# praveer13/zest

Measured on AMD Instinct MI355X. Metric: aggregate pull GB/s + P2P ratio, Llama-3.1-70B at 1/2/4/8 MI355X peers, higher is better.
Workload: dtype bf16

## Files before the change

### csrc/gpu/compress.hip

```cpp
#include <hip/hip_runtime.h>

#include <cstdint>
#include <cstdlib>

#include "zgpu.h"

namespace {

constexpr int kWave = 64;
constexpr int kWavesPerBlock = 4;
constexpr int kTabLog = 12;
constexpr uint32_t kTab = 1u << kTabLog;

__device__ __forceinline__ uint32_t lane_id() { return threadIdx.x & (kWave - 1); }

__device__ __forceinline__ uint32_t load_u32(const uint8_t* p) {
  const uintptr_t a = reinterpret_cast<uintptr_t>(p);
  const uint32_t k = uint32_t(a & 3);
  const uint32_t* w = reinterpret_cast<const uint32_t*>(a & ~uintptr_t(3));
  const uint32_t w0 = w[0];
  return k == 0 ? w0 : __builtin_amdgcn_alignbyte(w[1], w0, k);
}

__device__ __forceinline__ uint32_t put_len(uint8_t* o, uint32_t op, uint32_t r, uint32_t lane) {
  const uint32_t nff = r / 255;
  for (uint32_t i = lane; i < nff; i += kWave) o[op + i] = 0xFF;
  if (lane == 0) o[op + nff] = uint8_t(r - 255 * nff);
  return op + nff + 1;
}

__device__ __forceinline__ uint32_t emit(uint8_t* o, uint32_t op, const uint8_t* in, uint32_t lit0, uint32_t L,
                                         uint32_t off, uint32_t ml, uint32_t lane) {
  const uint32_t M = ml ? ml - 4 : 0;
  if (lane == 0) o[op] = uint8_t(((L < 15 ? L : 15) << 4) | (ml ? (M < 15 ? M : 15) : 0));
  ++op;
  if (L >= 15) op = put_len(o, op, L - 15, lane);
  for (uint32_t i = lane; i < L; i += kWave) o[op + i] = in[lit0 + i];
  op += L;
  if (ml) {
    if (lane == 0) {
      o[op] = uint8_t(off & 0xFF);
      o[op + 1] = uint8_t(off >> 8);
    }
    op += 2;
    if (M >= 15) op = put_len(o, op, M - 15, lane);
  }
  return op;
}

__global__ void __launch_bounds__(256) k_bg4_split(const uint8_t* __restrict__ data, const uint64_t* __restrict__ offs,
                                                   const uint32_t* __restrict__ lens, int n, uint8_t* __restrict__ out,
                                                   uint64_t slot) {
  const int c = __builtin_amdgcn_readfirstlane(int(blockIdx.x * kWavesPerBlock + (threadIdx.x >> 6)));
  if (c >= n) return;
  const uint32_t lane = lane_id(), len = lens[c];
  const uint8_t* s = data + offs[c];
  uint8_t* d = out + uint64_t(c) * slot;
  const uint32_t q = len >> 2, r = len & 3;
  const uint32_t g1 = q + (r > 0), g2 = g1 + q + (r > 1), g3 = g2 + q + (r > 2);
  for (uint32_t i = lane; i < len; i += kWave) {
    const uint32_t g = i & 3, j = i >> 2;
    const uint32_t base = g == 0 ? 0u : g == 1 ? g1 : g == 2 ? g2 : g3;
    d[base + j] = s[i];
  }
}

__global__ void __launch_bounds__(256) k_lz4_compress_v1(const uint8_t* __restrict__ data, const uint64_t* __restrict__ offs,
                                                      const uint32_t* __restrict__ lens, int n, uint64_t in_slot,
                                                      uint8_t* __restrict__ out, uint64_t out_slot,
                                                      uint32_t* __restrict__ out_len, uint32_t hc64, uint32_t hc256) {
  __shared__ unsigned long long tabs[kWavesPerBlock][kTab];
  const int wave = __builtin_amdgcn_readfirstlane(int(threadIdx.x >> 6));
  const int c = __builtin_amdgcn_readfirstlane(int(blockIdx.x * kWavesPerBlock + wave));
  if (c >= n) return;
  const uint32_t lane = lane_id();
  unsigned long long* tab = tabs[wave];
  for (uint32_t i = lane; i < kTab; i += kWave) tab[i] = 0;
  __builtin_amdgcn_wave_barrier();
  const uint32_t len = lens[c];
  const uint8_t* in = in_slot ? data + uint64_t(c) * in_slot : data + offs[c];
  uint8_t* o = out + uint64_t(c) * out_slot;
  uint32_t op = 11, ip = 0, anchor = 0;
  const uint32_t mend = len > 5 ? len - 5 : 0;
  while (ip + 12 <= len) {
    const uint32_t p = ip + lane;
    const bool ok = p + 12 <= len;
    const uint32_t v = ok ? load_u32(in + p) : 0;
    const uint32_t h = (v * 2654435761u) >> (32 - kTabLog);
    const unsigned long long e = ok ? tab[h] : 0ull;
    uint32_t cand = uint32_t(e >> 32) - 1;
    bool hit = ok && e != 0 && uint32_t(e) == v && cand < p && p - cand <= 65535u;
    uint32_t near = 0;
    for (int d = 32; d >= 1; --d) {
      const uint32_t u = __shfl_up(v, d, kWave);
      if (lane >= uint32_t(d) && u == v) near = d;
    }
    if (ok && near) {
      cand = p - near;
      hit = true;
    }
    const unsigned long long mask = __ballot(hit);
    const uint32_t passed = mask ? uint32_t(__builtin_ctzll(mask)) + 1 : uint32_t(kWave);
    __builtin_amdgcn_wave_barrier();
    if (ok && lane < passed) atomicMax(&tab[h], (static_cast<unsigned long long>(p + 1) << 32) | v);
    if (!mask) {
      ip += kWave;
      continue;
    }
    const int j = __builtin_ctzll(mask);
    uint32_t mp = ip + uint32_t(j);
    uint32_t mc = uint32_t(__builtin_amdgcn_readlane(int(cand), j));
    while (true) {
      const uint32_t room = (mp - anchor) < mc ? (mp - anchor) : mc;
      if (room == 0) break;
      const uint32_t k = lane + 1;
      const bool eq = k <= room && in[mp - k] == in[mc - k];
      const unsigned long long ne = __ballot(!eq);
      const uint32_t b = ne ? uint32_t(__builtin_ctzll(ne)) : uint32_t(kWave);
      mp -= b;
      mc -= b;
      if (b < uint32_t(kWave)) break;
    }
    const uint32_t maxlen = mend - mp;
    uint32_t ml = 4 + (ip + uint32_t(j) - mp);
    while (ml < maxlen) {
      const uint32_t k = ml + lane;
      const bool eq = k < maxlen && in[mc + k] == in[mp + k];
      const unsigned long long ne = __ballot(!eq);
      if (ne) {
        ml += uint32_t(__builtin_ctzll(ne));
        break;
      }
      ml += kWave;
    }
    if (ml > maxlen) ml = maxlen;
    op = emit(o, op, in, anchor, mp - anchor, mp - mc, ml, lane);
    ip = mp + ml;
    anchor = ip;
  }
  op = emit(o, op, in, anchor, len - anchor, 0, 0, lane);
  const uint32_t total = op + 4;
  if (total >= len) {
    if (lane == 0) out_len[c] = 0;
    return;
  }
  if (lane == 0) {
    const uint32_t bs = op - 11;
    const bool small = len <= 65536;
    const uint8_t hdr[11] = {0x04, 0x22, 0x4D, 0x18, 0x60, uint8_t(small ? 0x40 : 0x50),
                             uint8_t(small ? hc64 : hc256), uint8_t(bs), uint8_t(bs >> 8), uint8_t(bs >> 16),
                             uint8_t(bs >> 24)};
    for (int i = 0; i < 11; ++i) o[i] = hdr[i];
    for (int i = 0; i < 4; ++i) o[op + i] = 0;
    out_len[c] = total;
  }
}

constexpr uint32_t kTagBits = 14;
constexpr uint32_t kTagMask = (1u << kTagBits) - 1;
constexpr uint32_t kRing = 4096;
constexpr uint32_t kRingMask = kRing - 1;
constexpr uint32_t kFlush = 2048;
constexpr uint32_t kHdr = 11;

struct Staged {
  uint8_t* ring;
  uint8_t* g;
  uint32_t flushed;
};

__device__ __forceinline__ void ring_write(Staged& o, uint32_t end, uint32_t lane) {
  __builtin_amdgcn_wave_barrier();
  for (uint32_t pos = o.flushed + lane; pos < end; pos += kWave)
    if (pos >= kHdr) o.g[pos] = o.ring[pos & kRingMask];
  __builtin_amdgcn_wave_barrier();
}

__device__ __forceinline__ void maybe_flush(Staged& o, uint32_t op, uint32_t lane) {
  while (op - o.flushed >= kFlush) {
    ring_write(o, o.flushed + kFlush, lane);
    o.flushed += kFlush;
  }
}

__device__ __forceinline__ uint32_t put_len_s(Staged& o, uint32_t op, uint32_t r, uint32_t lane) {
  const uint32_t nff = r / 255;
  for (uint32_t i = lane; i < nff; i += kWave) o.ring[(op + i) & kRingMask] = 0xFF;
  if (lane == 0) o.ring[(op + nff) & kRingMask] = uint8_t(r - 255 * nff);
  return op + nff + 1;
}

__device__ __forceinline__ uint32_t emit_s(Staged& o, uint32_t op, const uint8_t* in, uint32_t lit0, uint32_t L,
                                           uint32_t off, uint32_t ml, uint32_t lane) {
  const uint32_t M = ml ? ml - 4 : 0;
  maybe_flush(o, op, lane);
  if (lane == 0) o.ring[op & kRingMask] = uint8_t(((L < 15 ? L : 15) << 4) | (ml ? (M < 15 ? M : 15) : 0));
  ++op;
  if (L >= 15) op = put_len_s(o, op, L - 15, lane);
  for (uint32_t b = 0; b < L; b += 1024) {
    maybe_flush(o, op + b, lane);
    const uint32_t n = L - b < 1024 ? L - b : 1024;
    for (uint32_t i = lane; i < n; i += kWave) o.ring[(op + b + i) & kRingMask] = in[lit0 + b + i];
  }
  op += L;
  if (ml) {
    maybe_flush(o, op, lane);
    if (lane == 0) {
      o.ring[op & kRingMask] = uint8_t(off & 0xFF);
      o.ring[(op + 1) & kRingMask] = uint8_t(off >> 8);
    }
    op += 2;
    if (M >= 15) op = put_len_s(o, op, M - 15, lane);
  }
  return op;
}

__global__ void __launch_bounds__(256) k_lz4_compress(const uint8_t* __restrict__ data, const uint64_t* __restrict__ offs,
                                                      const uint32_t* __restrict__ lens, int n, uint64_t in_slot,
                                                      uint8_t* __restrict__ out, uint64_t out_slot,
                                                      uint32_t* __restrict__ out_len, uint32_t hc64, uint32_t hc256) {
  __shared__ uint32_t tabs[kWavesPerBlock][kTab];
  __shared__ uint8_t rings[kWavesPerBlock][kRing];
  const int wave = __builtin_amdgcn_readfirstlane(int(threadIdx.x >> 6));
  const int c = __builtin_amdgcn_readfirstlane(int(blockIdx.x * kWavesPerBlock + wave));
  if (c >= n) return;
  const uint32_t lane = lane_id();
  uint32_t* tab = tabs[wave];
  for (uint32_t i = lane; i < kTab; i += kWave) tab[i] = 0;
  __builtin_amdgcn_wave_barrier();
  const uint32_t len = lens[c];
  const uint8_t* in = in_slot ? data + uint64_t(c) * in_slot : data + offs[c];
  Staged o{rings[wave], out + uint64_t(c) * out_slot, 0};
  uint32_t op = kHdr, ip = 0, anchor = 0;
  const uint32_t mend = len > 5 ? len - 5 : 0;
  while (ip + 12 <= len) {
    const uint32_t p = ip + lane;
    const bool ok = p + 12 <= len;
    const uint32_t v = ok ? load_u32(in + p) : 0;
    const uint32_t hv = v * 2654435761u;
    const uint32_t h = hv >> (32 - kTabLog);
    const uint32_t tag = hv & kTagMask;
    const uint32_t e = ok ? tab[h] : 0u;
    uint32_t cand = (e >> kTagBits) - 1;
    bool hit = ok && e != 0 && (e & kTagMask) == tag && cand < p && p - cand <= 65535u;
    if (hit) hit = load_u32(in + cand) == v;
    uint32_t near = 0;
    for (int d = 32; d >= 1; --d) {
      const uint32_t u = __shfl_up(v, d, kWave);
      if (lane >= uint32_t(d) && u == v) near = d;
    }
    if (ok && near) {
      cand = p - near;
      hit = true;
    }
    const unsigned long long mask = __ballot(hit);
    const uint32_t passed = mask ? uint32_t(__builtin_ctzll(mask)) + 1 : uint32_t(kWave);
    __builtin_amdgcn_wave_barrier();
    if (ok && lane < passed) atomicMax(&tab[h], ((p + 1) << kTagBits) | tag);
    if (!mask) {
      ip += kWave;
      continue;
    }
    const int j = __builtin_ctzll(mask);
    uint32_t mp = ip + uint32_t(j);
    uint32_t mc = uint32_t(__builtin_amdgcn_readlane(int(cand), j));
    while (true) {
      const uint32_t room = (mp - anchor) < mc ? (mp - anchor) : mc;
      if (room == 0) break;
      const uint32_t k = lane + 1;
      const bool eq = k <= room && in[mp - k] == in[mc - k];
      const unsigned long long ne = __ballot(!eq);
      const uint32_t b = ne ? uint32_t(__builtin_ctzll(ne)) : uint32_t(kWave);
      mp -= b;
      mc -= b;
      if (b < uint32_t(kWave)) break;
    }
    const uint32_t maxlen = mend - mp;
    uint32_t ml = 4 + (ip + uint32_t(j) - mp);
    while (ml < maxlen) {
      const uint32_t k = ml + lane;
      const bool eq = k < maxlen && in[mc + k] == in[mp + k];
      const unsigned long long ne = __ballot(!eq);
      if (ne) {
        ml += uint32_t(__builtin_ctzll(ne));
        break;
      }
      ml += kWave;
    }
    if (ml > maxlen) ml = maxlen;
    op = emit_s(o, op, in, anchor, mp - anchor, mp - mc, ml, lane);
    ip = mp + ml;
    anchor = ip;
  }
  op = emit_s(o, op, in, anchor, len - anchor, 0, 0, lane);
  const uint32_t total = op + 4;
  if (total >= len) {
    if (lane == 0) out_len[c] = 0;
    return;
  }
  maybe_flush(o, op, lane);
  if (lane < 4) o.ring[(op + lane) & kRingMask] = 0;
  ring_write(o, total, lane);
  if (lane == 0) {
    const uint32_t bs = op - kHdr;
    const bool small = len <= 65536;
    const uint8_t hdr[kHdr] = {0x04, 0x22, 0x4D, 0x18, 0x60, uint8_t(small ? 0x40 : 0x50),
                               uint8_t(small ? hc64 : hc256), uint8_t(bs), uint8_t(bs >> 8), uint8_t(bs >> 16),
                               uint8_t(bs >> 24)};
    for (uint32_t i = 0; i < kHdr; ++i) o.g[i] = hdr[i];
    out_len[c] = total;
  }
}

bool compress_v1() {
  const char* e = getenv("ZG_COMPRESS");
  return e && e[0] == 'v' && e[1] == '1';
}

__global__ void __launch_bounds__(256) k_pack_frames(const uint64_t* __restrict__ src, const uint32_t* __restrict__ clen,
                                                     const uint32_t* __restrict__ ulen, const uint8_t* __restrict__ scheme,
                                                     const uint64_t* __restrict__ out_off, int n, uint8_t* __restrict__ out) {
  const int c = __builtin_amdgcn_readfirstlane(int(blockIdx.x * kWavesPerBlock + (threadIdx.x >> 6)));
  if (c >= n) return;
  const uint32_t lane = lane_id(), cl = clen[c], ul = ulen[c];
  uint8_t* d = out + out_off[c];
  if (lane < 8) {
    const uint32_t b = lane == 0 ? 0u : lane < 4 ? (cl >> (8 * (lane - 1))) & 0xFF
                                  : lane == 4 ? scheme[c] : (ul >> (8 * (lane - 5))) & 0xFF;
    d[lane] = uint8_t(b);
  }
  const uint8_t* s = reinterpret_cast<const uint8_t*>(src[c]);
  for (uint32_t i = lane; i < cl; i += kWave) d[8 + i] = s[i];
}

}

extern "C" {

hipError_t zg_compress_chunks(const uint8_t* data, const uint64_t* offs, const uint32_t* lens, int n, int bg4,
                              uint8_t* scratch, uint64_t in_slot, uint8_t* out, uint64_t out_slot, uint32_t* out_len,
                              uint32_t hc64, uint32_t hc256, hipStream_t stream) {
  if (n <= 0) return hipSuccess;
  const dim3 grid((n + kWavesPerBlock - 1) / kWavesPerBlock);
  auto* kern = compress_v1() ? k_lz4_compress_v1 : k_lz4_compress;
  if (bg4) {
    hipLaunchKernelGGL(k_bg4_split, grid, dim3(256), 0, stream, data, offs, lens, n, scratch, in_slot);
    hipLaunchKernelGGL(kern, grid, dim3(256), 0, stream, scratch, offs, lens, n, in_slot, out, out_slot, out_len,
                       hc64, hc256);
  } else {
    hipLaunchKernelGGL(kern, grid, dim3(256), 0, stream, data, offs, lens, n, uint64_t(0), out, out_slot, out_len,
                       hc64, hc256);
  }
  return hipGetLastError();
}

hipError_t zg_pack_frames(const uint64_t* src, const uint32_t* clen, const uint32_t* ulen, const uint8_t* scheme,
                          const uint64_t* out_off, int n, uint8_t* out, hipStream_t stream) {
  if (n <= 0) return hipSuccess;
  hipLaunchKernelGGL(k_pack_frames, dim3((n + kWavesPerBlock - 1) / kWavesPerBlock), dim3(256), 0, stream, src, clen,
                     ulen, scheme, out_off, n, out);
  return hipGetLastError();
}

}
```

Baseline: 63.18.

## Stage LZ4 input in LDS window, reuse wave scans after matches, vectorize byte-group split

```diff
diff --git a/csrc/gpu/compress.hip b/csrc/gpu/compress.hip
--- a/csrc/gpu/compress.hip
+++ b/csrc/gpu/compress.hip
@@ -48,6 +48,11 @@
   return op;
 }
 
+typedef uint32_t __attribute__((aligned(1))) dword_any;
+struct __attribute__((packed, aligned(1))) Dwords4 {
+  uint32_t v[4];
+};
+
 __global__ void __launch_bounds__(256) k_bg4_split(const uint8_t* __restrict__ data, const uint64_t* __restrict__ offs,
                                                    const uint32_t* __restrict__ lens, int n, uint8_t* __restrict__ out,
                                                    uint64_t slot) {
@@ -58,7 +63,18 @@
   uint8_t* d = out + uint64_t(c) * slot;
   const uint32_t q = len >> 2, r = len & 3;
   const uint32_t g1 = q + (r > 0), g2 = g1 + q + (r > 1), g3 = g2 + q + (r > 2);
-  for (uint32_t i = lane; i < len; i += kWave) {
+  const uint32_t nv = len >> 4;
+  for (uint32_t t = lane; t < nv; t += kWave) {
+    const Dwords4 a = *reinterpret_cast<const Dwords4*>(s + 16 * t);
+#pragma unroll
+    for (uint32_t g = 0; g < 4; ++g) {
+      const uint32_t base = g == 0 ? 0u : g == 1 ? g1 : g == 2 ? g2 : g3;
+      const uint32_t x = ((a.v[0] >> (8 * g)) & 0xFF) | (((a.v[1] >> (8 * g)) & 0xFF) << 8) |
+                         (((a.v[2] >> (8 * g)) & 0xFF) << 16) | (((a.v[3] >> (8 * g)) & 0xFF) << 24);
+      *reinterpret_cast<dword_any*>(d + base + 4 * t) = x;
+    }
+  }
+  for (uint32_t i = 16 * nv + lane; i < len; i += kWave) {
     const uint32_t g = i & 3, j = i >> 2;
     const uint32_t base = g == 0 ? 0u : g == 1 ? g1 : g == 2 ? g2 : g3;
     d[base + j] = s[i];
@@ -158,20 +174,135 @@
 
 constexpr uint32_t kTagBits = 14;
 constexpr uint32_t kTagMask = (1u << kTagBits) - 1;
-constexpr uint32_t kRing = 4096;
+constexpr uint32_t kRing = 2048;
 constexpr uint32_t kRingMask = kRing - 1;
-constexpr uint32_t kFlush = 2048;
+constexpr uint32_t kFlush = 1024;
+constexpr uint32_t kPiece = 512;
 constexpr uint32_t kHdr = 11;
+constexpr uint32_t kWin = 2048;
+constexpr uint32_t kWinDw = kWin / 4;
+constexpr uint32_t kBlk = 1024;
+constexpr uint32_t kAhead = 96;
+
+struct Win {
+  uint32_t* w;
+  const uint32_t* g;
+  uint32_t nd;
+  uint32_t lo, hi;
+  uint32_t pre[4];
+};
+
+__device__ __forceinline__ uint32_t glob_dw(const Win& s, int32_t d) {
+  const int32_t last = int32_t(s.nd) - 1;
+  const int32_t k = d < 0 ? 0 : d > last ? last : d;
+  const uint32_t x = *reinterpret_cast<const uint32_t*>(reinterpret_cast<const uint8_t*>(s.g) + (uint32_t(k) << 2));
+  return k == d ? x : 0u;
+}
+
+__device__ __forceinline__ uint32_t glob_u32(const Win& s, uint32_t q) {
+  const int32_t d = int32_t(q >> 2);
+  return __builtin_amdgcn_alignbyte(glob_dw(s, d + 1), glob_dw(s, d), q & 3);
+}
+
+__device__ __forceinline__ uint32_t glob_u8(const Win& s, uint32_t q) {
+  return (glob_dw(s, int32_t(q >> 2)) >> (8 * (q & 3))) & 0xFF;
+}
+
+__device__ __forceinline__ uint32_t win_dw(const Win& s, uint32_t d) { return s.w[d & (kWinDw - 1)]; }
+
+__device__ __forceinline__ uint32_t win_u32(const Win& s, uint32_t q) {
+  const uint32_t d = q >> 2;
+  return __builtin_amdgcn_alignbyte(win_dw(s, d + 1), win_dw(s, d), q & 3);
+}
+
+__device__ __forceinline__ uint32_t win_u8(const Win& s, uint32_t q) {
+  return reinterpret_cast<const uint8_t*>(s.w)[q & (kWin - 1)];
+}
+
+__device__ __forceinline__ void win_prefetch(Win& s, uint32_t lane) {
+#pragma unroll
+  for (uint32_t i = 0; i < 4; ++i) {
+    const uint32_t d = (s.hi >> 2) + lane + kWave * i;
+    s.pre[i] = d < s.nd ? s.g[d] : 0u;
+  }
+}
+
+__device__ __forceinline__ void win_need(Win& s, uint32_t q_ip, uint32_t q_end, uint32_t lane) {
+  if (q_end <= s.hi) return;
+  if (q_ip >= s.hi + kBlk) {
+    s.hi = (q_ip - 4) & ~(kBlk - 1);
+    s.lo = s.hi;
+    win_prefetch(s, lane);
+  }
+  __builtin_amdgcn_wave_barrier();
+  while (s.hi < q_end) {
+#pragma unroll
+    for (uint32_t i = 0; i < 4; ++i) s.w[((s.hi >> 2) + lane + kWave * i) & (kWinDw - 1)] = s.pre[i];
+    s.hi += kBlk;
+    if (s.hi - s.lo > kWin) s.lo = s.hi - kWin;
+    win_prefetch(s, lane);
+  }
+  __builtin_amdgcn_wave_barrier();
+}
+
+struct Span {
+  uint32_t b;
+  uint32_t f[4];
+};
+
+__device__ __forceinline__ Span span_from(const uint32_t (&c)[6], uint32_t k) {
+  Span r;
+  r.b = __builtin_amdgcn_alignbyte(c[1], c[0], k);
+#pragma unroll
+  for (int i = 0; i < 4; ++i) r.f[i] = __builtin_amdgcn_alignbyte(c[i + 2], c[i + 1], k);
+  return r;
+}
+
+__device__ __forceinline__ Span span_win(const Win& s, uint32_t q) {
+  const uint32_t d = uint32_t((int32_t(q) - 4) >> 2);
+  uint32_t c[6];
+#pragma unroll
+  for (uint32_t i = 0; i < 6; ++i) c[i] = win_dw(s, d + i);
+  return span_from(c, q & 3);
+}
+
+__device__ __forceinline__ Span span_any(const Win& s, uint32_t q) {
+  const int32_t d = (int32_t(q) - 4) >> 2;
+  if (int32_t(q) - 4 >= int32_t(s.lo) && uint32_t(d + 6) * 4 <= s.hi) return span_win(s, q);
+  uint32_t c[6];
+#pragma unroll
+  for (int i = 0; i < 6; ++i) c[i] = glob_dw(s, d + i);
+  return span_from(c, q & 3);
+}
+
+__device__ __forceinline__ Span span_of_lane(const Span& x, uint32_t l) {
+  Span r;
+  r.b = uint32_t(__builtin_amdgcn_readlane(int(x.b), int(l)));
+#pragma unroll
+  for (int i = 0; i < 4; ++i) r.f[i] = uint32_t(__builtin_amdgcn_readlane(int(x.f[i]), int(l)));
+  return r;
+}
 
 struct Staged {
   uint8_t* ring;
   uint8_t* g;
   uint32_t flushed;
+  bool g_aligned;
 };
 
 __device__ __forceinline__ void ring_write(Staged& o, uint32_t end, uint32_t lane) {
   __builtin_amdgcn_wave_barrier();
-  for (uint32_t pos = o.flushed + lane; pos < end; pos += kWave)
+  uint32_t from = o.flushed;
+  if (o.g_aligned) {
+    const uint32_t end4 = end & ~3u;
+    const uint32_t* r4 = reinterpret_cast<const uint32_t*>(o.ring);
+    for (uint32_t pos = from + 4 * lane; pos < end4; pos += 4 * kWave) {
+      if (pos >= 12) *reinterpret_cast<uint32_t*>(o.g + pos) = r4[(pos & kRingMask) >> 2];
+      else if (pos == 8) o.g[kHdr] = o.ring[kHdr];
+    }
+    if (end4 > from) from = end4;
+  }
+  for (uint32_t pos = from + lane; pos < end; pos += kWave)
     if (pos >= kHdr) o.g[pos] = o.ring[pos & kRingMask];
   __builtin_amdgcn_wave_barrier();
 }
@@ -190,18 +321,38 @@
   return op + nff + 1;
 }
 
-__device__ __forceinline__ uint32_t emit_s(Staged& o, uint32_t op, const uint8_t* in, uint32_t lit0, uint32_t L,
-                                           uint32_t off, uint32_t ml, uint32_t lane) {
+__device__ __forceinline__ void put_literals(Staged& o, uint32_t op, const Win& s, uint32_t q, uint32_t L,
+                                             uint32_t lane) {
+  const bool in_win = q >= s.lo && q + L <= s.hi;
+  uint32_t* r4 = reinterpret_cast<uint32_t*>(o.ring);
+  for (uint32_t b = 0; b < L; b += kPiece) {
+    maybe_flush(o, op + b, lane);
+    const uint32_t n = L - b < kPiece ? L - b : kPiece;
+    const uint32_t dst = op + b, src = q + b;
+    uint32_t done = 0;
+    if (n > kWave) {
+      const uint32_t head = (0u - dst) & 3;
+      if (lane < head) o.ring[(dst + lane) & kRingMask] = uint8_t(in_win ? win_u8(s, src + lane) : glob_u8(s, src + lane));
+      const uint32_t body = (n - head) & ~3u;
+      for (uint32_t i = 4 * lane; i < body; i += 4 * kWave) {
+        const uint32_t x = src + head + i;
+        r4[((dst + head + i) & kRingMask) >> 2] = in_win ? win_u32(s, x) : glob_u32(s, x);
+      }
+      done = head + body;
+    }
+    for (uint32_t i = done + lane; i < n; i += kWave)
+      o.ring[(dst + i) & kRingMask] = uint8_t(in_win ? win_u8(s, src + i) : glob_u8(s, src + i));
+  }
+}
+
+__device__ __forceinline__ uint32_t emit_s(Staged& o, uint32_t op, const Win& s, uint32_t q, uint32_t L, uint32_t off,
+                                           uint32_t ml, uint32_t lane) {
   const uint32_t M = ml ? ml - 4 : 0;
   maybe_flush(o, op, lane);
   if (lane == 0) o.ring[op & kRingMask] = uint8_t(((L < 15 ? L : 15) << 4) | (ml ? (M < 15 ? M : 15) : 0));
   ++op;
   if (L >= 15) op = put_len_s(o, op, L - 15, lane);
-  for (uint32_t b = 0; b < L; b += 1024) {
-    maybe_flush(o, op + b, lane);
-    const uint32_t n = L - b < 1024 ? L - b : 1024;
-    for (uint32_t i = lane; i < n; i += kWave) o.ring[(op + b + i) & kRingMask] = in[lit0 + b + i];
-  }
+  put_literals(o, op, s, q, L, lane);
   op += L;
   if (ml) {
     maybe_flush(o, op, lane);
@@ -220,79 +371,168 @@
                                                       uint8_t* __restrict__ out, uint64_t out_slot,
                                                       uint32_t* __restrict__ out_len, uint32_t hc64, uint32_t hc256) {
   __shared__ uint32_t tabs[kWavesPerBlock][kTab];
-  __shared__ uint8_t rings[kWavesPerBlock][kRing];
+  __shared__ uint32_t wins[kWavesPerBlock][kWinDw];
+  __shared__ uint32_t rings[kWavesPerBlock][kRing / 4];
   const int wave = __builtin_amdgcn_readfirstlane(int(threadIdx.x >> 6));
   const int c = __builtin_amdgcn_readfirstlane(int(blockIdx.x * kWavesPerBlock + wave));
   if (c >= n) return;
   const uint32_t lane = lane_id();
+  const uint32_t len = lens[c];
+  const uint8_t* in = in_slot ? data + uint64_t(c) * in_slot : data + offs[c];
+  const uint32_t sh = uint32_t(reinterpret_cast<uintptr_t>(in) & 3);
+  Win W{wins[wave], reinterpret_cast<const uint32_t*>(in - sh), len ? (sh + len + 3) >> 2 : 0u, 0, 0, {}};
+  win_prefetch(W, lane);
   uint32_t* tab = tabs[wave];
   for (uint32_t i = lane; i < kTab; i += kWave) tab[i] = 0;
   __builtin_amdgcn_wave_barrier();
-  const uint32_t len = lens[c];
-  const uint8_t* in = in_slot ? data + uint64_t(c) * in_slot : data + offs[c];
-  Staged o{rings[wave], out + uint64_t(c) * out_slot, 0};
+  uint8_t* g = out + uint64_t(c) * out_slot;
+  Staged o{reinterpret_cast<uint8_t*>(rings[wave]), g, 0, (reinterpret_cast<uintptr_t>(g) & 3) == 0};
   uint32_t op = kHdr, ip = 0, anchor = 0;
   const uint32_t mend = len > 5 ? len - 5 : 0;
   while (ip + 12 <= len) {
+    win_need(W, ip + sh, ip + sh + kAhead, lane);
     const uint32_t p = ip + lane;
     const bool ok = p + 12 <= len;
-    const uint32_t v = ok ? load_u32(in + p) : 0;
+    const uint32_t v = ok ? win_u32(W, p + sh) : 0;
     const uint32_t hv = v * 2654435761u;
     const uint32_t h = hv >> (32 - kTabLog);
     const uint32_t tag = hv & kTagMask;
-    const uint32_t e = ok ? tab[h] : 0u;
-    uint32_t cand = (e >> kTagBits) - 1;
-    bool hit = ok && e != 0 && (e & kTagMask) == tag && cand < p && p - cand <= 65535u;
-    if (hit) hit = load_u32(in + cand) == v;
+    const uint32_t entry = ((p + 1) << kTagBits) | tag;
+    uint32_t e = ok ? tab[h] : 0u;
     uint32_t near = 0;
-    for (int d = 32; d >= 1; --d) {
+#pragma unroll
+    for (uint32_t d = 32; d >= 1; --d) {
       const uint32_t u = __shfl_up(v, d, kWave);
-      if (lane >= uint32_t(d) && u == v) near = d;
-    }
-    if (ok && near) {
-      cand = p - near;
-      hit = true;
-    }
-    const unsigned long long mask = __ballot(hit);
-    const uint32_t passed = mask ? uint32_t(__builtin_ctzll(mask)) + 1 : uint32_t(kWave);
-    __builtin_amdgcn_wave_barrier();
-    if (ok && lane < passed) atomicMax(&tab[h], ((p + 1) << kTagBits) | tag);
-    if (!mask) {
+      if (lane >= d && u == v) near = d;
+    }
+    if (!ok) near = 0;
+    bool th = ok && e != 0 && (e & kTagMask) == tag && (e >> kTagBits) - 1 < p && p - ((e >> kTagBits) - 1) <= 65535u;
+    if (!(__ballot(th) | __ballot(near != 0))) {
+      __builtin_amdgcn_wave_barrier();
+      if (ok) atomicMax(&tab[h], entry);
       ip += kWave;
       continue;
     }
-    const int j = __builtin_ctzll(mask);
-    uint32_t mp = ip + uint32_t(j);
-    uint32_t mc = uint32_t(__builtin_amdgcn_readlane(int(cand), j));
+    const Span ms = span_win(W, p + sh);
+    Span cs{};
+    if (th) cs = span_any(W, (e >> kTagBits) - 1 + sh);
+    unsigned long long dead = 0;
+    uint32_t start = 0;
     while (true) {
-      const uint32_t room = (mp - anchor) < mc ? (mp - anchor) : mc;
-      if (room == 0) break;
-      const uint32_t k = lane + 1;
-      const bool eq = k <= room && in[mp - k] == in[mc - k];
-      const unsigned long long ne = __ballot(!eq);
-      const uint32_t b = ne ? uint32_t(__builtin_ctzll(ne)) : uint32_t(kWave);
-      mp -= b;
-      mc -= b;
-      if (b < uint32_t(kWave)) break;
-    }
-    const uint32_t maxlen = mend - mp;
-    uint32_t ml = 4 + (ip + uint32_t(j) - mp);
-    while (ml < maxlen) {
-      const uint32_t k = ml + lane;
-      const bool eq = k < maxlen && in[mc + k] == in[mp + k];
-      const unsigned long long ne = __ballot(!eq);
-      if (ne) {
-        ml += uint32_t(__builtin_ctzll(ne));
+      const uint32_t cand = (e >> kTagBits) - 1;
+      th = ok && e != 0 && (e & kTagMask) == tag && cand < p && p - cand <= 65535u;
+      unsigned long long tm = __ballot(th) & ~dead & (~0ull << start);
+      const unsigned long long nm = __ballot(near != 0 && near + start <= lane);
+      uint32_t j, mc = 0;
+      Span s{};
+      while (true) {
+        const uint32_t jt = tm ? uint32_t(__builtin_ctzll(tm)) : uint32_t(kWave);
+        const uint32_t jn = nm ? uint32_t(__builtin_ctzll(nm)) : uint32_t(kWave);
+        if (jn <= jt) {
+          j = jn;
+          if (j < uint32_t(kWave)) {
+            const uint32_t nj = uint32_t(__builtin_amdgcn_readlane(int(near), int(j)));
+            mc = ip + j - nj;
+            s = span_of_lane(ms, j - nj);
+          }
+          break;
+        }
+        mc = uint32_t(__builtin_amdgcn_readlane(int(cand), int(jt)));
+        s = mc >= ip ? span_of_lane(ms, mc - ip) : span_of_lane(cs, jt);
+        if (s.f[0] == uint32_t(__builtin_amdgcn_readlane(int(v), int(jt)))) {
+          j = jt;
+          break;
+        }
+        dead |= 1ull << jt;
+        tm &= tm - 1;
+      }
+      if (j == uint32_t(kWave)) {
+        if (start == 0) {
+          __builtin_amdgcn_wave_barrier();
+          if (ok) atomicMax(&tab[h], entry);
+          ip += kWave;
+        } else {
+          ip += start;
+        }
         break;
       }
-      ml += kWave;
-    }
-    if (ml > maxlen) ml = maxlen;
-    op = emit_s(o, op, in, anchor, mp - anchor, mp - mc, ml, lane);
-    ip = mp + ml;
-    anchor = ip;
-  }
-  op = emit_s(o, op, in, anchor, len - anchor, 0, 0, lane);
+      __builtin_amdgcn_wave_barrier();
+      if (lane >= start && lane <= j) atomicMax(&tab[h], entry);
+      const Span m = span_of_lane(ms, j);
+      const uint32_t hp = ip + j;
+      uint32_t mp = hp;
+      {
+        const uint32_t room = (mp - anchor) < mc ? (mp - anchor) : mc;
+        const uint32_t x = s.b ^ m.b;
+        const uint32_t eq = x ? uint32_t(__builtin_clz(x)) >> 3 : 4u;
+        const uint32_t b = eq < room ? eq : room;
+        mp -= b;
+        mc -= b;
+        if (eq == 4 && room > 4) {
+          while (true) {
+            const uint32_t room2 = (mp - anchor) < mc ? (mp - anchor) : mc;
+            if (room2 == 0) break;
+            const uint32_t k = lane + 1;
+            const bool same = k <= room2 && glob_u8(W, mp - k + sh) == glob_u8(W, mc - k + sh);
+            const unsigned long long ne = __ballot(!same);
+            const uint32_t b2 = ne ? uint32_t(__builtin_ctzll(ne)) : uint32_t(kWave);
+            mp -= b2;
+            mc -= b2;
+            if (b2 < uint32_t(kWave)) break;
+          }
+        }
+      }
+      const uint32_t maxlen = mend - mp;
+      const unsigned long long x0 = (static_cast<unsigned long long>(s.f[1] ^ m.f[1]) << 32) | (s.f[0] ^ m.f[0]);
+      const unsigned long long x1 = (static_cast<unsigned long long>(s.f[3] ^ m.f[3]) << 32) | (s.f[2] ^ m.f[2]);
+      const uint32_t eqf = x0 ? uint32_t(__builtin_ctzll(x0)) >> 3 : 8u + (x1 ? uint32_t(__builtin_ctzll(x1)) >> 3 : 8u);
+      uint32_t ml = (hp - mp) + eqf;
+      if (eqf == 16) {
+        while (ml < maxlen) {
+          const uint32_t k = ml + 4 * lane;
+          const uint32_t x = k < maxlen ? glob_u32(W, mc + k + sh) ^ glob_u32(W, mp + k + sh) : 1u;
+          const uint32_t same = x ? uint32_t(__builtin_ctz(x)) >> 3 : 4u;
+          const unsigned long long ne = __ballot(same < 4);
+          if (ne) {
+            const int f = __builtin_ctzll(ne);
+            ml += 4 * uint32_t(f) + uint32_t(__builtin_amdgcn_readlane(int(same), f));
+            break;
+          }
+          ml += 4 * kWave;
+        }
+      }
+      if (ml > maxlen) ml = maxlen;
+      const uint32_t nlit = mp - anchor;
+      if (anchor == ip + start && nlit < 15) {
+        maybe_flush(o, op, lane);
+        const uint32_t r = (lane - start) & (kWave - 1), M = ml - 4, off = mp - mc;
+        uint32_t x = v, at = op + 1 + r;
+        if (r == nlit) x = (nlit << 4) | (M < 15 ? M : 15), at = op;
+        if (r == nlit + 1) x = off, at = op + r;
+        if (r == nlit + 2) x = off >> 8, at = op + r;
+        if (r < nlit + 3) o.ring[at & kRingMask] = uint8_t(x);
+        op += nlit + 3;
+        if (M >= 15) op = put_len_s(o, op, M - 15, lane);
+      } else {
+        op = emit_s(o, op, W, anchor + sh, nlit, mp - mc, ml, lane);
+      }
+      const uint32_t ip2 = mp + ml, nstart = ip2 - ip;
+      anchor = ip2;
+      if (nstart >= uint32_t(kWave) || j - start >= 8 || ip2 + 12 > len) {
+        ip = ip2;
+        break;
+      }
+      for (uint32_t k = start; k <= j; ++k) {
+        const uint32_t hk = uint32_t(__builtin_amdgcn_readlane(int(h), int(k)));
+        const uint32_t ek = uint32_t(__builtin_amdgcn_readlane(int(entry), int(k)));
+        const bool upd = h == hk && ek > e;
+        if (upd) e = ek;
+        dead &= ~__ballot(upd);
+      }
+      start = nstart;
+    }
+  }
+  op = emit_s(o, op, W, anchor + sh, len - anchor, 0, 0, lane);
   const uint32_t total = op + 4;
   if (total >= len) {
     if (lane == 0) out_len[c] = 0;
```

After: 63.07, median of 2. About the same (-0.2%).
